# neka-nat/probreg

Hardware: NVIDIA H100
Metric: cpd_em_iterations_per_sec (higher is better)
Workload: dtype f32

## Files before the change

### probreg_b200/csrc/cpd_b200.cu

```cuda
#include "cpd_b200.h"
#include "kernels.cuh"
#include "lowrank.cuh"
#include "gram_i8.cuh"
#include "bcpd.cuh"
#include "gmmtree.cuh"
#include "l2dist.cuh"
#include "ocsvm.cuh"
#include "lattice.cuh"
#include "batch.cuh"

#include <cub/device/device_radix_sort.cuh>
#ifdef CPD_HOST_EMU
#include "emu_nccl.h"
#include "emu_solver.h"
#endif

#include <dlfcn.h>
#include <math.h>
#include <stdarg.h>
#include <stdio.h>
#include <stdlib.h>
#include <string.h>

#include <algorithm>
// ... 205 lines not shown
    DevBuf<float4> d_srcP, d_tgtP, d_tgtQ;
    DevBuf<P1Part> d_part1;
    DevBuf<double> d_part2;
    DevBuf<double> d_pt1, d_p1, d_pxc, d_px;
    DevBuf<double> d_mom_src, d_mom_tgt, d_mom, d_sums;
    DevBuf<DevState> d_state;
    DevState h_state;
    PinBuf<PinStage> pin;
    DevBuf<double> d_frame;
    PinBuf<double> h_stats;
    Event stats_ev, copy_ev;
    int stats_pending = 0;
    long long stats_count[2] = {0, 0};
    bool origin_given = false;
    int it1 = 0, it2 = 0, j1 = 1, j2 = 1, g1 = 1, g2 = 1;
    DevBuf<float4> d_sbox, d_tbox, d_ssub, d_tsub;
    DevBuf<float> d_omax, d_omax_sub;
    bool cull_on = true, cull_active = false;
    double extent = 0.0;
    DevBuf<int4> d_work1, d_work2;
    DevBuf<int> d_slots1, d_slots2;
    bool have_source = false, have_target = false, have_state = false, prepared = false;
    nccl_comm comm = nullptr;
    int world = 1, rank = 0;
    DevBuf<int> d_perm_src, d_perm_tgt, d_idx_tmp;
    DevBuf<unsigned> d_codes, d_codes_out;
    DevBuf<unsigned char> d_sort_tmp;
    DevBuf<double> d_outN, d_outM;
    DevBuf<float> d_G;
    DevBuf<double> d_W, d_A, d_B, d_ts2, d_nrpart;
    DevBuf<int64_t> d_ipiv;
    DevBuf<int> d_info;
    DevBuf<unsigned char> d_work;
// ... 63 lines not shown
    DevBuf<unsigned char> d_flush;
    std::vector<Event> pool;
};

namespace {
constexpr int STATE_RING = 8;
inline void drop_graph(cpd_ctx* h) {
#ifndef CPD_HOST_EMU
    h->em_graph.reset();
#endif
    (void)h;
}

inline unsigned blocks_for(long long n) { return (unsigned)((n + THREADS - 1) / THREADS); }

struct WorkList {
    std::vector<int4> items;
    std::vector<int> tile_slots;
    int max_slots = 1;
};
WorkList build_work(int ntiles, int nunits, int slots, double last_cost, double overhead) {
    const double OVERHEAD = overhead;
    WorkList w;
    nunits = std::max(1, nunits);
    auto cost_of = [&](int t) { return t == ntiles - 1 ? last_cost : 1.0; };
    auto span_of = [&](int t, int j) { return cost_of(t) * (double)((nunits + j - 1) / j) + OVERHEAD; };
    int best_j = 1;
    double best = 1e300;
    for (int j = 1; j <= nunits; ++j) {
        const long long items = (long long)ntiles * j;
// ... 121 lines not shown
        const double* t = h->h_stats.p + 9;
        if (!h->origin_given) for (int a = 0; a < 3; ++a) h->h_state.cx[a] = t[a] / (double)h->stats_count[1];
        h->extent = std::max(t[6] - t[3], std::max(t[7] - t[4], t[8] - t[5]));
    }
    h->stats_pending = 0;
    return CPD_OK;
}

int prepare(cpd_ctx* h) {
    TRY(ensure_stats(h));
    if (h->prepared) return CPD_OK;
    if (!h->have_source || !h->have_target) return fail(CPD_ERR_STATE, "source and target must both be set");
    h->it1 = (int)((h->n + ITILE1 - 1) / ITILE1);
    h->it2 = (int)((h->m + ITILE2 - 1) / ITILE2);
    const long long in_last = h->n - (long long)(h->it1 - 1) * ITILE1;
    const int live = (int)((in_last + 32 * RI1 - 1) / (32 * RI1));
    double last_cost = live < THREADS / 32 ? std::max(0.6, live / (double)(THREADS / 32)) : 1.0;
    if (const char* e = getenv("CPD_B200_PLAN_LAST_COST")) { const double v = atof(e); if (v > 0.0 && v <= 1.0) last_cost = v; }
    WorkList w1;
    if (const char* e = getenv("CPD_B200_PLAN_UNIT"); e && !strcmp(e, "stage")) {
        w1 = build_work(h->it1, (int)(h->mpad / P1_STAGE), h->slots1, last_cost, 0.5);
        for (int4& it : w1.items) { it.y *= P1_STAGE / SUB; it.z *= P1_STAGE / SUB; }
    } else {
        w1 = build_work(h->it1, (int)(h->mpad / SUB), h->slots1, last_cost, 0.5 * (P1_STAGE / SUB));
    }
    const WorkList w2 = build_work(h->it2, (int)(h->npad / P2_STAGE), h->slots2, 1.0, 0.5);
    h->j1 = w1.max_slots; h->g1 = (int)w1.items.size();
    h->j2 = w2.max_slots; h->g2 = (int)w2.items.size();
    TRY(h->d_work1.alloc(w1.items.size()));
    TRY(h->d_work2.alloc(w2.items.size()));
    TRY(h->d_slots1.alloc(w1.tile_slots.size()));
    TRY(h->d_slots2.alloc(w2.tile_slots.size()));
    CU(cudaMemcpyAsync(h->d_work1.p, w1.items.data(), w1.items.size() * sizeof(int4), cudaMemcpyHostToDevice, h->stream));
    CU(cudaMemcpyAsync(h->d_work2.p, w2.items.data(), w2.items.size() * sizeof(int4), cudaMemcpyHostToDevice, h->stream));
    CU(cudaMemcpyAsync(h->d_slots1.p, w1.tile_slots.data(), w1.tile_slots.size() * sizeof(int), cudaMemcpyHostToDevice, h->stream));
    CU(cudaMemcpyAsync(h->d_slots2.p, w2.tile_slots.data(), w2.tile_slots.size() * sizeof(int), cudaMemcpyHostToDevice, h->stream));
    CU(cudaStreamSynchronize(h->stream));
    TRY(h->d_sbox.alloc((size_t)(h->mpad / P1_STAGE) * 2));
    TRY(h->d_tbox.alloc((size_t)(h->npad / P2_STAGE) * 2));
    TRY(h->d_omax.alloc((size_t)(h->npad / P2_STAGE)));
    TRY(h->d_ssub.alloc((size_t)(h->mpad / SUB) * 2));
    TRY(h->d_tsub.alloc((size_t)(h->npad / SUB) * 2));
    TRY(h->d_omax_sub.alloc((size_t)(h->npad / SUB)));
    const size_t need1 = (size_t)h->j1 * h->n, need2 = (size_t)h->j2 * h->m * 4;
    TRY(h->d_part1.reserve(need1));
    TRY(h->d_part2.reserve(need2));
    const size_t ms = (size_t)blocks_for(h->m) * MOM_SRC, mt = (size_t)blocks_for(h->npad) * MOM_TGT;
    TRY(h->d_mom_src.reserve(ms));
    TRY(h->d_mom_tgt.reserve(mt));
    h->prepared = true;
    drop_graph(h);
    return CPD_OK;
}

int allreduce(cpd_ctx* h, double* buf, size_t count) {
// ... 7 lines not shown
}

int launch_estep(cpd_ctx* h, const double* d_sigma2, const double* d_w, const double* d_ts) {
    TRY(prepare(h));
    const long long cover = std::max(h->mpad, h->n);
    mark(h, 0);
    pack_kernel<<<blocks_for(cover), THREADS, 0, h->stream>>>(h->d_state.p, d_sigma2, h->d_yc.p, d_ts, h->d_xc.p, h->m, h->mpad,
                                                              h->n, h->d_srcP.p, h->d_tgtP.p);
    mark(h, 1);
    const bool cull = h->cull_on && h->cull_active;
    const int nst1 = (int)(h->mpad / P1_STAGE);
    stage_bbox_kernel<<<(unsigned)nst1, THREADS, 0, h->stream>>>(h->d_srcP.p, (int)h->m, P1_STAGE, h->d_sbox.p);
    h->launches += 1;
    const int nsub1 = (int)(h->mpad / SUB), nsub2 = (int)(h->npad / SUB);
    if (cull) {
        stage_bbox_kernel<<<(unsigned)(h->npad / P2_STAGE), THREADS, 0, h->stream>>>(h->d_tgtP.p, (int)h->n, P2_STAGE, h->d_tbox.p);
        sub_bbox_kernel<<<(unsigned)((nsub1 + 7) / 8), THREADS, 0, h->stream>>>(h->d_srcP.p, (int)h->m, nsub1, h->d_ssub.p);
        sub_bbox_kernel<<<(unsigned)((nsub2 + 7) / 8), THREADS, 0, h->stream>>>(h->d_tgtP.p, (int)h->n, nsub2, h->d_tsub.p);
        h->launches += 3;
    }
    const bool wgt = h->wgt_on;
    if (wgt) {
        weight_patch_kernel<<<blocks_for(h->m), THREADS, 0, h->stream>>>(h->d_la.p, h->m, h->d_srcP.p);
        h->launches += 1;
    }
#define CPD_PASS1(C, W) pass1_kernel<C, W><<<h->g1, THREADS, PASS1_SMEM, h->stream>>>(h->d_tgtP.p, (int)h->n, h->d_srcP.p, h->d_work1.p, h->d_part1.p, h->d_sbox.p, nst1, (C) ? h->d_ssub.p : nullptr)
    if (cull) { if (wgt) CPD_PASS1(true, true); else CPD_PASS1(true, false); }
    else { if (wgt) CPD_PASS1(false, true); else CPD_PASS1(false, false); }
#undef CPD_PASS1
    mark(h, 2);
    finalize1_kernel<<<blocks_for(h->npad), THREADS, 0, h->stream>>>(h->d_state.p, d_sigma2, d_w, h->d_part1.p, h->d_slots1.p, (int)h->n,
                                                                     h->d_tgtP.p, h->d_tgtQ.p, h->npad, h->d_pt1.p, h->d_mom_tgt.p,
                                                                     wgt ? h->d_log2c.p : nullptr);
    mark(h, 3);
    if (cull) {
        stage_omax_kernel<<<(unsigned)(h->npad / P2_STAGE), THREADS, 0, h->stream>>>(h->d_tgtQ.p, h->d_omax.p);
        sub_omax_kernel<<<(unsigned)((nsub2 + 7) / 8), THREADS, 0, h->stream>>>(h->d_tgtQ.p, nsub2, h->d_omax_sub.p);
        h->launches += 2;
    }
#define CPD_PASS2(C, W) pass2_kernel<C, W><<<h->g2, THREADS, PASS2_SMEM, h->stream>>>(h->d_srcP.p, (int)h->m, h->d_tgtQ.p, h->d_work2.p, h->d_part2.p, (C) ? h->d_tbox.p : nullptr, (C) ? h->d_omax.p : nullptr, (C) ? h->d_tsub.p : nullptr, (C) ? h->d_omax_sub.p : nullptr)
    if (cull) { if (wgt) CPD_PASS2(true, true); else CPD_PASS2(true, false); }
    else { if (wgt) CPD_PASS2(false, true); else CPD_PASS2(false, false); }
#undef CPD_PASS2
    mark(h, 4);
    finalize2_kernel<<<blocks_for(h->m), THREADS, 0, h->stream>>>(h->d_state.p, d_sigma2, h->d_part2.p, h->d_slots2.p, (int)h->m, h->d_yc.p,
                                                                  d_ts, h->d_p1.p, h->d_pxc.p, h->d_mom_src.p);
    mark(h, 5);
    mark(h, 6);
    KCHECK();
    h->launches += 5;
    return CPD_OK;
}

int read_params(cpd_ctx* h, cpd_params* out) {
    const DevState& s = h->pin.p->state;
    CU(cudaMemcpyAsync(&h->pin.p->state, h->d_state.p, sizeof(DevState), cudaMemcpyDeviceToHost, h->stream));
    CU(cudaStreamSynchronize(h->stream));
    if (s.err)
        return fail(CPD_ERR_STATE, "a peer rank did not deliver its moments within the P2P exchange timeout");
    const int d = h->dim;
    for (int i = 0; i < 9; ++i) out->lin[i] = 0.0;
    for (int i = 0; i < d; ++i)
        for (int j = 0; j < d; ++j) out->lin[i * d + j] = s.lin[3 * i + j];
    for (int i = 0; i < 3; ++i) out->t[i] = (i < d) ? s.t[i] : 0.0;
    out->scale = s.scale;
    out->sigma2 = s.sigma2;
    TRY(ensure_stats(h));
    h->cull_active = h->extent > 0.0 && 13.3 * sqrt(out->sigma2) < 0.25 * h->extent;
    out->q = s.q;
    out->n_p = s.n_p;
    return CPD_OK;
}
}

extern "C" int cpd_plan_work(int ntiles, int nunits, int slots, double last_tile_cost, int* items ,
                             int capacity, int* n_items, int* max_slots) {
    if (ntiles < 1 || nunits < 1 || slots < 1 || !(last_tile_cost > 0.0 && last_tile_cost <= 1.0) || !n_items || !max_slots)
        return fail(CPD_ERR_ARG, "bad argument");
    const WorkList w = build_work(ntiles, nunits, slots, last_tile_cost, 0.5 * (P1_STAGE / SUB));
    *n_items = (int)w.items.size();
    *max_slots = w.max_slots;
    if (items) {
        if (capacity < (int)w.items.size()) return fail(CPD_ERR_ARG, "capacity %d < %d work items", capacity, (int)w.items.size());
// ... 20 lines not shown
        return fail(CPD_ERR_CUDA, "device %d is sm_%d%d; this library is built for sm_90a (Hopper) only", device, prop.major, prop.minor);
    std::unique_ptr<cpd_ctx> h(new cpd_ctx());
    h->device = device;
    h->dim = dim;
    h->sm_count = prop.multiProcessorCount;
    if (stream) h->stream = (cudaStream_t)stream;
    else { CU(cudaStreamCreateWithFlags(&h->owned_stream.s, cudaStreamNonBlocking)); h->stream = h->owned_stream.s; }
    CU(cudaFuncSetAttribute(pass1_kernel<false, false>, cudaFuncAttributeMaxDynamicSharedMemorySize, PASS1_SMEM));
    CU(cudaFuncSetAttribute(pass2_kernel<false, false>, cudaFuncAttributeMaxDynamicSharedMemorySize, PASS2_SMEM));
    CU(cudaFuncSetAttribute(pass1_kernel<true, false>, cudaFuncAttributeMaxDynamicSharedMemorySize, PASS1_SMEM));
    CU(cudaFuncSetAttribute(pass2_kernel<true, false>, cudaFuncAttributeMaxDynamicSharedMemorySize, PASS2_SMEM));
    CU(cudaFuncSetAttribute(pass1_kernel<false, true>, cudaFuncAttributeMaxDynamicSharedMemorySize, PASS1_SMEM));
    CU(cudaFuncSetAttribute(pass2_kernel<false, true>, cudaFuncAttributeMaxDynamicSharedMemorySize, PASS2_SMEM));
    CU(cudaFuncSetAttribute(pass1_kernel<true, true>, cudaFuncAttributeMaxDynamicSharedMemorySize, PASS1_SMEM));
    CU(cudaFuncSetAttribute(pass2_kernel<true, true>, cudaFuncAttributeMaxDynamicSharedMemorySize, PASS2_SMEM));
    int occ1 = 0, occ2 = 0;
    CU(cudaOccupancyMaxActiveBlocksPerMultiprocessor(&occ1, pass1_kernel<false, false>, THREADS, PASS1_SMEM));
    CU(cudaOccupancyMaxActiveBlocksPerMultiprocessor(&occ2, pass2_kernel<false, false>, THREADS, PASS2_SMEM));
    h->slots1 = h->sm_count * std::max(1, occ1);
    h->slots2 = h->sm_count * std::max(1, occ2);
    TRY(h->d_state.alloc(1));
    TRY(h->d_mom.alloc((size_t)MOM_PAD));
    TRY(h->pin.alloc(1));
    TRY(h->d_frame.alloc(16));
    TRY(h->h_stats.alloc(18));
    CU(cudaEventCreateWithFlags(&h->stats_ev.e, cudaEventDisableTiming));
    CU(cudaEventCreateWithFlags(&h->copy_ev.e, cudaEventDisableTiming));
    CU(cudaEventCreate(&h->ev0.e));
    CU(cudaEventCreate(&h->ev1.e));
    for (Event& e : h->sev) CU(cudaEventCreate(&e.e));
    { const char* e = getenv("CPD_B200_NO_CULL"); h->cull_on = !(e && e[0] == '1'); }
    { const char* e = getenv("CPD_B200_NO_GRAPH"); h->graph_on = !(e && e[0] == '1'); }
    memset(&h->h_state, 0, sizeof(DevState));
    h->h_state.dim = dim;
    h->h_state.scale = 1.0;
    h->h_state.lin[0] = h->h_state.lin[4] = h->h_state.lin[8] = 1.0;
    h->h_state.update_scale = 1;
    TRY(upload_state(h.get()));
    *out = h.release();
    return CPD_OK;
}

extern "C" void cpd_destroy(cpd_ctx* h) {
    if (!h) return;
    cudaSetDevice(h->device);
    cudaStreamSynchronize(h->stream);
// ... 83 lines not shown
    CU(cudaSetDevice(h->device));
    DevState& s = h->h_state;
    const int d = h->dim;
    for (int i = 0; i < 3; ++i)
        for (int j = 0; j < 3; ++j) s.lin[3 * i + j] = (i < d && j < d) ? init->lin[i * d + j] : (i == j ? 1.0 : 0.0);
    for (int i = 0; i < 3; ++i) s.t[i] = (i < d) ? init->t[i] : 0.0;
    s.scale = (tf_kind == CPD_TF_RIGID) ? init->scale : 1.0;
    s.sigma2 = init->sigma2;
    s.q = init->q;
    s.n_p = 0.0;
    s.w = w;
    s.tf_kind = tf_kind;
    s.update_scale = update_scale ? 1 : 0;
    s.dim = d;
    TRY(ensure_stats(h));
    h->cull_active = h->extent > 0.0 && 13.3 * sqrt(init->sigma2) < 0.25 * h->extent;
    h->have_state = true;
    return upload_state(h);
}

namespace {
int em_step_launches(cpd_ctx* h) {
    TRY(launch_estep(h, &h->d_state.p->sigma2, &h->d_state.p->w, nullptr));
    const int nbs = (int)blocks_for(h->m), nbt = (int)blocks_for(h->npad);
    if (h->d_p2p.p) {
        moments_p2p_kernel<<<1, 256, 0, h->stream>>>(h->d_state.p, h->d_mom_src.p, nbs, RM_SRC, h->d_mom_tgt.p, nbt, RM_TGT, h->d_mom.p,
                                                     h->d_p2p.p);
        h->launches += 1;
    } else if (h->comm) {
        moments_kernel<0><<<1, 256, 0, h->stream>>>(h->d_state.p, h->d_mom_src.p, nbs, RM_SRC, h->d_mom_tgt.p, nbt, RM_TGT, h->d_mom.p);
        TRY(allreduce(h, h->d_mom.p, MOM_PAD));
// ... 69 lines not shown
    if (iters_run) *iters_run = it;
    return CPD_OK;
}

extern "C" int cpd_estep(cpd_ctx* h, const double* t_source, double sigma2, double w, double* pt1, double* p1, double* px, double* n_p) {
    if (!h || !t_source) return fail(CPD_ERR_ARG, "null argument");
    if (!(sigma2 > 0.0)) return fail(CPD_ERR_ARG, "sigma2 must be positive, got %g", sigma2);
    if (!(w >= 0.0 && w < 1.0)) return fail(CPD_ERR_ARG, "w must be in [0, 1), got %g", w);
    if (!h->have_source || !h->have_target) return fail(CPD_ERR_STATE, "source and target must both be set");
    CU(cudaSetDevice(h->device));
    TRY(h->d_raw.reserve((size_t)h->m * 3));
    TRY(upload_cloud(h, t_source, h->m, h->d_raw.p));
    gather3_kernel<<<blocks_for(h->m), THREADS, 0, h->stream>>>(h->d_raw.p, h->d_perm_src.p, h->m, 0.0, 0.0, 0.0, h->d_ts.p);
    h->launches += 1;
    TRY(ensure_stats(h));
    h->cull_active = h->extent > 0.0 && 13.3 * sqrt(sigma2) < 0.25 * h->extent;
    h->pin.p->es[0] = sigma2;
    h->pin.p->es[1] = w;
    CU(cudaMemcpyAsync(&h->d_state.p->es_sigma2, h->pin.p->es, 2 * sizeof(double), cudaMemcpyHostToDevice, h->stream));
    TRY(launch_estep(h, &h->d_state.p->es_sigma2, &h->d_state.p->es_w, h->d_ts.p));
    if (h->comm) {
        TRY(allreduce(h, h->d_p1.p, (size_t)h->m));
        TRY(allreduce(h, h->d_pxc.p, (size_t)h->m * 3));
    }
    return cpd_last_estep(h, pt1, p1, px, n_p);
}

namespace {
int bcpd_weights(cpd_ctx* h, const double* alpha, const double* sdiag, const int* perm, const double* ssw) {
    const long long m = h->m;
    const unsigned nb = blocks_for(m);
// ... 30 lines not shown
    }
    if (!any_weight) return fail(CPD_ERR_ARG, "every source has zero weight");
    TRY(ensure_weight_buffers(h));
    h->pin.p->bc_ssw[0] = scale;
    h->pin.p->bc_ssw[1] = sigma2;
    h->pin.p->bc_ssw[2] = w;
    CU(cudaMemcpyAsync(h->d_bc_es.p, h->pin.p->bc_ssw, 3 * sizeof(double), cudaMemcpyHostToDevice, h->stream));
    CU(cudaMemcpyAsync(h->d_outM.p, alpha, (size_t)m * sizeof(double), cudaMemcpyHostToDevice, h->stream));
    CU(cudaMemcpyAsync(h->d_outM.p + m, sigma_diag, (size_t)m * sizeof(double), cudaMemcpyHostToDevice, h->stream));
    TRY(bcpd_weights(h, h->d_outM.p, h->d_outM.p + m, h->d_perm_src.p, h->d_bc_es.p));
    TRY(h->d_raw.reserve((size_t)m * 3));
    TRY(upload_cloud(h, t_source, m, h->d_raw.p));
    gather3_kernel<<<blocks_for(m), THREADS, 0, h->stream>>>(h->d_raw.p, h->d_perm_src.p, m, 0.0, 0.0, 0.0, h->d_ts.p);
    h->launches += 1;
    TRY(ensure_stats(h));
    h->cull_active = h->extent > 0.0 && 13.3 * sqrt(sigma2) < 0.25 * h->extent;
    h->pin.p->es[0] = sigma2;
    h->pin.p->es[1] = w;
    CU(cudaMemcpyAsync(&h->d_state.p->es_sigma2, h->pin.p->es, 2 * sizeof(double), cudaMemcpyHostToDevice, h->stream));
    h->wgt_on = true;
    const int r = launch_estep(h, &h->d_state.p->es_sigma2, &h->d_state.p->es_w, h->d_ts.p);
    h->wgt_on = false;
    TRY(r);
    if (h->comm) {
        TRY(allreduce(h, h->d_p1.p, (size_t)m));
        TRY(allreduce(h, h->d_pxc.p, (size_t)m * 3));
    }
    return cpd_last_estep(h, nu_d, nu, px, n_p);
}

extern "C" int cpd_last_estep(cpd_ctx* h, double* pt1, double* p1, double* px, double* n_p) {
// ... 78 lines not shown
```

### probreg_b200/csrc/kernels.cuh

```cuda
#pragma once
#include <cuda_runtime.h>
#include <stdint.h>

namespace cpd {

#ifndef CPD_RI1
#define CPD_RI1 4
#endif
#ifndef CPD_RI2
#define CPD_RI2 4
#endif
#ifndef CPD_MINB1
#define CPD_MINB1 2
#endif
#ifndef CPD_MINB2
#define CPD_MINB2 2
#endif
#ifndef CPD_UNROLL1
#define CPD_UNROLL1 4
#endif
#ifndef CPD_UNROLL2
#define CPD_UNROLL2 4
#endif
#ifndef CPD_SUB
#define CPD_SUB 64
#endif
#ifndef CPD_GRP
#define CPD_GRP 8
#endif
constexpr int UNROLL1 = CPD_UNROLL1, UNROLL2 = CPD_UNROLL2;
constexpr int THREADS = 256;
constexpr int RI1 = CPD_RI1, RI2 = CPD_RI2;
constexpr int ITILE1 = THREADS * RI1, ITILE2 = THREADS * RI2;
#ifndef CPD_P1_STAGE
#define CPD_P1_STAGE 512
#endif
#ifndef CPD_P2_STAGE
#define CPD_P2_STAGE 512
#endif
constexpr int P1_STAGE = CPD_P1_STAGE;
constexpr int P2_STAGE = CPD_P2_STAGE;
static_assert(P1_STAGE % 256 == 0 && P2_STAGE % 256 == 0 && P1_STAGE >= 256 && P2_STAGE >= 256, "stage sizes are multiples of 256");
constexpr int P1_REC = 16, P2_REC = 32;
#ifndef CPD_NSTAGE
#define CPD_NSTAGE 3
#endif
constexpr int NSTAGE = CPD_NSTAGE;
constexpr int P1_STAGE_BYTES = P1_STAGE * P1_REC, P2_STAGE_BYTES = P2_STAGE * P2_REC;
// ... 195 lines not shown
        }
        srcP[i] = o;
    }
    if (i < n) {
        tgtP[i] = make_float4((float)(sk * xc[3 * i]), (float)(sk * xc[3 * i + 1]), (float)(sk * xc[3 * i + 2]), 0.0f);
    }
}

__global__ void __launch_bounds__(THREADS)
weight_patch_kernel(const float* __restrict__ la, long long m, float4* __restrict__ srcP) {
    const long long i = (long long)blockIdx.x * THREADS + threadIdx.x;
    if (i < m) srcP[i].w = la[i];
}

constexpr float CULL_GAP = 130.0f;
__global__ void __launch_bounds__(THREADS)
stage_bbox_kernel(const float4* __restrict__ pts, int n, int blk, float4* __restrict__ box) {
    __shared__ float sh[6][THREADS / 32];
    const int b = blockIdx.x;
    float lo[3] = {3.0e38f, 3.0e38f, 3.0e38f}, hi[3] = {-3.0e38f, -3.0e38f, -3.0e38f};
    for (int i = b * blk + threadIdx.x; i < min(n, (b + 1) * blk); i += THREADS) {
        const float4 p = pts[i];
        lo[0] = fminf(lo[0], p.x); lo[1] = fminf(lo[1], p.y); lo[2] = fminf(lo[2], p.z);
        hi[0] = fmaxf(hi[0], p.x); hi[1] = fmaxf(hi[1], p.y); hi[2] = fmaxf(hi[2], p.z);
    }
    const int lane = threadIdx.x & 31, wid = threadIdx.x >> 5;
#pragma unroll
    for (int a = 0; a < 3; ++a) {
#pragma unroll
        for (int o = 16; o > 0; o >>= 1) {
// ... 2 lines not shown
        }
        if (lane == 0) { sh[a][wid] = lo[a]; sh[3 + a][wid] = hi[a]; }
    }
    __syncthreads();
    if (threadIdx.x == 0) {
        float l[3], h[3];
        for (int a = 0; a < 3; ++a) {
            l[a] = sh[a][0]; h[a] = sh[3 + a][0];
            for (int w = 1; w < THREADS / 32; ++w) { l[a] = fminf(l[a], sh[a][w]); h[a] = fmaxf(h[a], sh[3 + a][w]); }
        }
        box[2 * b] = make_float4(l[0], l[1], l[2], 0.f);
        box[2 * b + 1] = make_float4(h[0], h[1], h[2], 0.f);
    }
}
__global__ void __launch_bounds__(THREADS)
stage_omax_kernel(const float4* __restrict__ tgtQ, float* __restrict__ omax) {
    __shared__ float sh[THREADS / 32];
    const int b = blockIdx.x;
    float m = 3.0e38f;
    for (int i = threadIdx.x; i < P2_STAGE; i += THREADS) m = fminf(m, tgtQ[2 * ((size_t)b * P2_STAGE + i)].w);
#pragma unroll
    for (int o = 16; o > 0; o >>= 1) m = fminf(m, __shfl_xor_sync(0xffffffffu, m, o));
    if ((threadIdx.x & 31) == 0) sh[threadIdx.x >> 5] = m;
    __syncthreads();
    if (threadIdx.x == 0) {
        for (int w = 1; w < THREADS / 32; ++w) m = fminf(m, sh[w]);
        omax[b] = -m;
    }
}
__global__ void __launch_bounds__(THREADS)
sub_bbox_kernel(const float4* __restrict__ pts, int n, int nsub, float4* __restrict__ box) {
    const int b = blockIdx.x * (THREADS / 32) + (threadIdx.x >> 5), lane = threadIdx.x & 31;
    if (b >= nsub) return;
    float lo[3] = {3.0e38f, 3.0e38f, 3.0e38f}, hi[3] = {-3.0e38f, -3.0e38f, -3.0e38f};
    for (int i = b * SUB + lane; i < min(n, (b + 1) * SUB); i += 32) {
        const float4 p = pts[i];
        lo[0] = fminf(lo[0], p.x); lo[1] = fminf(lo[1], p.y); lo[2] = fminf(lo[2], p.z);
        hi[0] = fmaxf(hi[0], p.x); hi[1] = fmaxf(hi[1], p.y); hi[2] = fmaxf(hi[2], p.z);
    }
#pragma unroll
    for (int a = 0; a < 3; ++a) {
#pragma unroll
        for (int o = 16; o > 0; o >>= 1) {
            lo[a] = fminf(lo[a], __shfl_xor_sync(0xffffffffu, lo[a], o));
            hi[a] = fmaxf(hi[a], __shfl_xor_sync(0xffffffffu, hi[a], o));
// ... 3 lines not shown
        box[2 * b] = make_float4(lo[0], lo[1], lo[2], 0.f);
        box[2 * b + 1] = make_float4(hi[0], hi[1], hi[2], 0.f);
    }
}
__global__ void __launch_bounds__(THREADS)
sub_omax_kernel(const float4* __restrict__ tgtQ, int nsub, float* __restrict__ omax) {
    const int b = blockIdx.x * (THREADS / 32) + (threadIdx.x >> 5), lane = threadIdx.x & 31;
    if (b >= nsub) return;
    float m = 3.0e38f;
    for (int i = lane; i < SUB; i += 32) m = fminf(m, tgtQ[2 * ((size_t)b * SUB + i)].w);
#pragma unroll
    for (int o = 16; o > 0; o >>= 1) m = fminf(m, __shfl_xor_sync(0xffffffffu, m, o));
    if (lane == 0) omax[b] = -m;
}
template <int RI>
__device__ __forceinline__ void warp_bbox(const float (&ax)[RI], const float (&ay)[RI], const float (&az)[RI], float* __restrict__ wbox) {
    float lo[3] = {3.0e38f, 3.0e38f, 3.0e38f}, hi[3] = {-3.0e38f, -3.0e38f, -3.0e38f};
#pragma unroll
    for (int r = 0; r < RI; ++r) {
        lo[0] = fminf(lo[0], ax[r]); hi[0] = fmaxf(hi[0], ax[r]);
        lo[1] = fminf(lo[1], ay[r]); hi[1] = fmaxf(hi[1], ay[r]);
        lo[2] = fminf(lo[2], az[r]); hi[2] = fmaxf(hi[2], az[r]);
    }
#pragma unroll
    for (int a = 0; a < 3; ++a) {
#pragma unroll
        for (int o = 16; o > 0; o >>= 1) {
            lo[a] = fminf(lo[a], __shfl_xor_sync(0xffffffffu, lo[a], o));
            hi[a] = fmaxf(hi[a], __shfl_xor_sync(0xffffffffu, hi[a], o));
        }
    }
// ... 9 lines not shown
    const float gz = fmaxf(0.f, fmaxf(blo.z - wbox[5], wbox[2] - bhi.z));
    return fmaf(gz, gz, fmaf(gy, gy, gx * gx)) * 0.9999f;
}

template <bool WGT>
__device__ __forceinline__ float pass1_t(const float ax, const float ay, const float az, const float no, const float4 b) {
    const float dx = __fsub_rn(ax, b.x), dy = __fsub_rn(ay, b.y), dz = __fsub_rn(az, b.z);
    float t = __fmaf_rn(dz, dz, __fmaf_rn(dy, dy, __fmaf_rn(dx, dx, no)));
    if (WGT) t = __fadd_rn(t, b.w);
    return t;
}
template <bool WGT>
__device__ __forceinline__ void pass1_sum(const float4* __restrict__ q, const float (&ax)[RI1], const float (&ay)[RI1],
                                          const float (&az)[RI1], const float (&no)[RI1], float (&Sc)[RI1], float (&Uc)[RI1]) {
    if (GRP > 0) {
#pragma unroll 1
        for (int g0 = 0; g0 < SUB; g0 += (GRP > 0 ? GRP : SUB)) {
            float gs[RI1], gu[RI1];
#pragma unroll
            for (int r = 0; r < RI1; ++r) {
#pragma unroll
                for (int jj = 0; jj < (GRP > 0 ? GRP : 1); ++jj) {
                    const float t = pass1_t<WGT>(ax[r], ay[r], az[r], no[r], q[g0 + jj]);
                    const float e = ex2(-t);
                    gs[r] = jj == 0 ? e : __fadd_rn(gs[r], e);
                    gu[r] = jj == 0 ? __fmul_rn(e, t) : __fmaf_rn(e, t, gu[r]);
                }
            }
#pragma unroll
            for (int r = 0; r < RI1; ++r) { Sc[r] = __fadd_rn(Sc[r], gs[r]); Uc[r] = __fadd_rn(Uc[r], gu[r]); }
        }
// ... 8 lines not shown
                Sc[r] = __fadd_rn(Sc[r], e);
                Uc[r] = __fmaf_rn(e, t, Uc[r]);
            }
        }
    }
}
template <bool WGT>
__device__ __forceinline__ float pass1_u(const float ax, const float ay, const float az, const float4 b) {
    const float dx = __fsub_rn(ax, b.x), dy = __fsub_rn(ay, b.y), dz = __fsub_rn(az, b.z);
    float u = __fmaf_rn(dz, dz, __fmaf_rn(dy, dy, __fmul_rn(dx, dx)));
    if (WGT) u = __fadd_rn(u, b.w);
    return u;
}

template <bool CULL, bool WGT>
__global__ void __launch_bounds__(THREADS, CPD_MINB1)
pass1_kernel(const float4* __restrict__ ipts, int ni, const float4* __restrict__ jrec, const int4* __restrict__ work,
             P1Part* __restrict__ part, const float4* __restrict__ sbox ,
             int nstages_total, const float4* __restrict__ ssub ) {
    __shared__ float wbox[THREADS / 32][8];
    CPD_DYN_SMEM(smraw);
    uint64_t* full = reinterpret_cast<uint64_t*>(smraw + NSTAGE * P1_STAGE_BYTES);
    const int tid = threadIdx.x;
    const int4 wk = work[blockIdx.x];
    constexpr int SPS = P1_STAGE / SUB;
    const int itile = wk.x, split = wk.w;
    const int st0 = wk.y / SPS, nst = (wk.z + SPS - 1) / SPS - st0;
    const int sc_first = wk.y - st0 * SPS, sc_last = wk.z - (st0 + nst - 1) * SPS;
    const unsigned char* jbytes = reinterpret_cast<const unsigned char*>(jrec);
    if (tid == 0) {
        for (int s = 0; s < NSTAGE; ++s) mbar_init(&full[s], 1);
        mbar_fence_init();
    }
    __syncthreads();
    if (tid == 0) {
// ... 1 lines not shown
            mbar_expect_tx(&full[s], P1_STAGE_BYTES);
            tma_load_1d(smraw + s * P1_STAGE_BYTES, jbytes + (size_t)(st0 + s) * P1_STAGE_BYTES, P1_STAGE_BYTES, &full[s]);
        }
    }
    if (itile * ITILE1 + (tid >> 5) * (32 * RI1) >= ni) return;
    float ax[RI1], ay[RI1], az[RI1], no[RI1];
    double S[RI1], SU[RI1];
#pragma unroll
    for (int r = 0; r < RI1; ++r) {
        int n = itile * ITILE1 + (tid >> 5) * (32 * RI1) + r * 32 + (tid & 31);
        n = n < ni ? n : ni - 1;
        const float4 p = ipts[n];
        ax[r] = p.x; ay[r] = p.y; az[r] = p.z;
        no[r] = -O_INIT;
    }
    float* const mybox = wbox[tid >> 5];
    warp_bbox<RI1>(ax, ay, az, mybox);
    {
        const int lane = tid & 31;
        float best = 3.0e38f;
        int bi = 0;
        for (int sidx = lane; sidx < nstages_total; sidx += 32) {
            const float g2 = box_gap2(mybox, sbox[2 * sidx], sbox[2 * sidx + 1]);
            if (g2 < best) { best = g2; bi = sidx; }
        }
#pragma unroll
        for (int o = 16; o > 0; o >>= 1) {
            const float ob = __shfl_xor_sync(0xffffffffu, best, o);
            const int oi = __shfl_xor_sync(0xffffffffu, bi, o);
            if (ob < best || (ob == best && oi < bi)) { best = ob; bi = oi; }
        }
        const float4* near = jrec + (size_t)bi * P1_STAGE;
        float cm[RI1];
#pragma unroll
        for (int r = 0; r < RI1; ++r) cm[r] = 3.0e38f;
#pragma unroll 4
        for (int jj = 0; jj < 128; ++jj) {
            const float4 b = near[jj];
#pragma unroll
            for (int r = 0; r < RI1; ++r) cm[r] = fminf(cm[r], pass1_u<WGT>(ax[r], ay[r], az[r], b));
        }
#pragma unroll
        for (int r = 0; r < RI1; ++r) no[r] = -fminf(O_INIT, floorf(cm[r]));
    }
    float omax_w = O_INIT;
    if (CULL) {
        float om = -3.0e38f;
#pragma unroll
        for (int r = 0; r < RI1; ++r) om = fmaxf(om, -no[r]);
#pragma unroll
        for (int o = 16; o > 0; o >>= 1) om = fmaxf(om, __shfl_xor_sync(0xffffffffu, om, o));
        omax_w = om;
    }
#pragma unroll
    for (int r = 0; r < RI1; ++r) { S[r] = 0.0; SU[r] = 0.0; }
    for (int it = 0; it < nst; ++it) {
        const int s = it % NSTAGE;
        mbar_wait(&full[s], (uint32_t)((it / NSTAGE) & 1));
        const float4* sp = reinterpret_cast<const float4*>(smraw + s * P1_STAGE_BYTES);
        bool skip = false;
        if (CULL) {
            const float4 blo = sbox[2 * (st0 + it)], bhi = sbox[2 * (st0 + it) + 1];
            skip = box_gap2(mybox, blo, bhi) - omax_w >= CULL_GAP;
        }
#pragma unroll 1
        for (int sc = (it == 0 ? sc_first : 0); sc < (skip ? 0 : (it == nst - 1 ? sc_last : SPS)); ++sc) {
            if (CULL) {
                const int sb = (st0 + it) * (P1_STAGE / SUB) + sc;
                if (box_gap2(mybox, ssub[2 * sb], ssub[2 * sb + 1]) - omax_w >= CULL_GAP) continue;
            }
            const float4* q = sp + sc * SUB;
            float Sc[RI1], Uc[RI1];
#pragma unroll
            for (int r = 0; r < RI1; ++r) { Sc[r] = 0.0f; Uc[r] = 0.0f; }
            pass1_sum<WGT>(q, ax, ay, az, no, Sc, Uc);
            bool bad = false;
#pragma unroll
            for (int r = 0; r < RI1; ++r) bad |= !(Sc[r] < TWO100);
            if (__any_sync(0xffffffffu, bad)) {
                float cm[RI1];
#pragma unroll
                for (int r = 0; r < RI1; ++r) cm[r] = 3.0e38f;
#pragma unroll UNROLL1
                for (int jj = 0; jj < SUB; ++jj) {
                    const float4 b = q[jj];
#pragma unroll
                    for (int r = 0; r < RI1; ++r) cm[r] = fminf(cm[r], pass1_u<WGT>(ax[r], ay[r], az[r], b));
                }
#pragma unroll
                for (int r = 0; r < RI1; ++r) {
                    const float o = -no[r], on = fminf(o, floorf(cm[r]));
                    const int sh = (int)fmaxf(on - o, -4000.0f);
                    S[r] = ldexp(S[r], sh); SU[r] = ldexp(SU[r], sh);
                    no[r] = -on;
                    Sc[r] = 0.0f; Uc[r] = 0.0f;
                }
                if (CULL) {
                    float om = -3.0e38f;
#pragma unroll
                    for (int r = 0; r < RI1; ++r) om = fmaxf(om, -no[r]);
#pragma unroll
                    for (int o = 16; o > 0; o >>= 1) om = fmaxf(om, __shfl_xor_sync(0xffffffffu, om, o));
                    omax_w = om;
                }
                pass1_sum<WGT>(q, ax, ay, az, no, Sc, Uc);
            }
#pragma unroll
            for (int r = 0; r < RI1; ++r) {
                S[r] += (double)Sc[r];
                SU[r] += (double)Uc[r] - (double)no[r] * (double)Sc[r];
            }
        }
        __syncthreads();
        if (tid == 0 && it + NSTAGE < nst) {
            mbar_expect_tx(&full[s], P1_STAGE_BYTES);
            tma_load_1d(smraw + s * P1_STAGE_BYTES, jbytes + (size_t)(st0 + it + NSTAGE) * P1_STAGE_BYTES, P1_STAGE_BYTES, &full[s]);
        }
    }
// ... 75 lines not shown
        finalize_column(log2S, c, lc, dead_shift, omin, SU, p1n, no, rnf, srr);
        pt1[i] = p1n;
        const float4 b = tgtP[i];
        v[0] = srr;
        v[1] = p1n;
        tgtQ[2 * (size_t)i] = make_float4(b.x, b.y, b.z, no);
        tgtQ[2 * (size_t)i + 1] = make_float4(rnf, 0.f, 0.f, 0.f);
    } else if (i < npad) {
        tgtQ[2 * (size_t)i] = make_float4(0.f, 0.f, 0.f, INFINITY);
        tgtQ[2 * (size_t)i + 1] = make_float4(0.f, 0.f, 0.f, 0.f);
    }
    block_reduce_store<RM_TGT>(v, mom_part + (size_t)blockIdx.x * RM_TGT);
}

template <bool CULL, bool WGT>
__global__ void __launch_bounds__(THREADS, CPD_MINB2)
pass2_kernel(const float4* __restrict__ ipts, int ni, const float4* __restrict__ jrec, const int4* __restrict__ work,
             double* __restrict__ part , const float4* __restrict__ tbox ,
             const float* __restrict__ omax_stage, const float4* __restrict__ tsub, const float* __restrict__ omax_sub) {
    __shared__ float wbox[THREADS / 32][8];
    CPD_DYN_SMEM(smraw);
    uint64_t* full = reinterpret_cast<uint64_t*>(smraw + NSTAGE * P2_STAGE_BYTES);
    const int tid = threadIdx.x;
    const int4 wk = work[blockIdx.x];
    const int itile = wk.x, st0 = wk.y, split = wk.w;
    const int nst = wk.z - wk.y;
    const unsigned char* jbytes = reinterpret_cast<const unsigned char*>(jrec);
    if (tid == 0) {
        for (int s = 0; s < NSTAGE; ++s) mbar_init(&full[s], 1);
        mbar_fence_init();
    }
    __syncthreads();
    if (tid == 0) {
        for (int s = 0; s < NSTAGE && s < nst; ++s) {
            mbar_expect_tx(&full[s], P2_STAGE_BYTES);
// ... 5 lines not shown
#pragma unroll
    for (int r = 0; r < RI2; ++r) {
        int m = itile * ITILE2 + (tid >> 5) * (32 * RI2) + r * 32 + (tid & 31);
        m = m < ni ? m : ni - 1;
        const float4 p = ipts[m];
        ax[r] = p.x; ay[r] = p.y; az[r] = p.z; al[r] = p.w;
    }
    float* const mybox = wbox[tid >> 5];
    if (CULL) warp_bbox<RI2>(ax, ay, az, mybox);
#pragma unroll
    for (int r = 0; r < RI2; ++r) { A1[r] = 0.0; AX[r] = 0.0; AY[r] = 0.0; AZ[r] = 0.0; }
    for (int it = 0; it < nst; ++it) {
        const int s = it % NSTAGE;
        mbar_wait(&full[s], (uint32_t)((it / NSTAGE) & 1));
        const float4* sp = reinterpret_cast<const float4*>(smraw + s * P2_STAGE_BYTES);
        bool skip = false;
        if (CULL) {
            const float4 blo = tbox[2 * (st0 + it)], bhi = tbox[2 * (st0 + it) + 1];
            skip = box_gap2(mybox, blo, bhi) - omax_stage[st0 + it] >= CULL_GAP;
        }
#pragma unroll 1
        for (int sc = 0; sc < (skip ? 0 : P2_STAGE / SUB); ++sc) {
            if (CULL) {
                const int sb = (st0 + it) * (P2_STAGE / SUB) + sc;
                if (box_gap2(mybox, tsub[2 * sb], tsub[2 * sb + 1]) - omax_sub[sb] >= CULL_GAP) continue;
            }
            const float4* q = sp + sc * (2 * SUB);
            float s1[RI2], sx[RI2], sy[RI2], sz[RI2];
#pragma unroll
            for (int r = 0; r < RI2; ++r) { s1[r] = 0.0f; sx[r] = 0.0f; sy[r] = 0.0f; sz[r] = 0.0f; }
            if (GRP > 0) {
#pragma unroll (CULL && WGT) ? 1 : 2
                for (int g0 = 0; g0 < SUB; g0 += (GRP > 0 ? GRP : SUB)) {
                    float g1[RI2], gx[RI2], gy[RI2], gz[RI2];
#pragma unroll
                    for (int jj = 0; jj < (GRP > 0 ? GRP : 1); ++jj) {
                        const float4 b = q[2 * (g0 + jj)];
                        const float rn = q[2 * (g0 + jj) + 1].x;
#pragma unroll
                        for (int r = 0; r < RI2; ++r) {
                            const float dx = __fsub_rn(ax[r], b.x), dy = __fsub_rn(ay[r], b.y), dz = __fsub_rn(az[r], b.z);
                            float t = __fmaf_rn(dz, dz, __fmaf_rn(dy, dy, __fmaf_rn(dx, dx, b.w)));
                            if (WGT) t = __fadd_rn(t, al[r]);
                            const float pr = __fmul_rn(ex2(-t), rn);
                            g1[r] = jj == 0 ? pr : __fadd_rn(g1[r], pr);
                            gx[r] = jj == 0 ? __fmul_rn(pr, dx) : __fmaf_rn(pr, dx, gx[r]);
                            gy[r] = jj == 0 ? __fmul_rn(pr, dy) : __fmaf_rn(pr, dy, gy[r]);
// ... 935 lines not shown
```

Baseline: 113.3.

## Cull CPD E-step at per-group sub-chunk granularity with decoupled tile sizes

Splits each pass1 warp's points into 128-point offset groups, each with its own bounding box, omax, and selective rebasing. Sub-chunk culling for a stage is now tested in parallel, one lane per sub-chunk, and combined with a warp ballot. This replaces the stage-level bbox/omax kernels and the per-iteration serial tests in both passes. Tile size is decoupled from thread count, slot counts come from launch bounds instead of the occupancy query, and the culling threshold becomes a tunable ratio. These changes aim to skip more far-field work and remove launches, at the cost of more per-group bookkeeping and a changed threshold (0.027 versus the old 0.25/13.3 ≈ 0.0188) that turns culling on in more cases.

Result: no change. 113.4 (median of 6 runs) (+0.1%).

```diff
diff --git a/probreg_b200/csrc/cpd_b200.cu b/probreg_b200/csrc/cpd_b200.cu
--- a/probreg_b200/csrc/cpd_b200.cu
+++ b/probreg_b200/csrc/cpd_b200.cu
@@ -243,9 +243,10 @@
     long long stats_count[2] = {0, 0};
     bool origin_given = false;
     int it1 = 0, it2 = 0, j1 = 1, j2 = 1, g1 = 1, g2 = 1;
-    DevBuf<float4> d_sbox, d_tbox, d_ssub, d_tsub;
-    DevBuf<float> d_omax, d_omax_sub;
+    DevBuf<float4> d_sbox, d_ssub, d_tsub;
+    DevBuf<float> d_omax_sub;
     bool cull_on = true, cull_active = false;
+    double cull_ratio = CULL_SIGMA_PER_EXTENT;
     double extent = 0.0;
     DevBuf<int4> d_work1, d_work2;
     DevBuf<int> d_slots1, d_slots2;
@@ -339,6 +340,10 @@
 
 inline unsigned blocks_for(long long n) { return (unsigned)((n + THREADS - 1) / THREADS); }
 
+inline void set_culling(cpd_ctx* h, double sigma2) {
+    h->cull_active = h->extent > 0.0 && sqrt(sigma2) < h->cull_ratio * h->extent;
+}
+
 struct WorkList {
     std::vector<int4> items;
     std::vector<int> tile_slots;
@@ -490,8 +495,8 @@
     h->it1 = (int)((h->n + ITILE1 - 1) / ITILE1);
     h->it2 = (int)((h->m + ITILE2 - 1) / ITILE2);
     const long long in_last = h->n - (long long)(h->it1 - 1) * ITILE1;
-    const int live = (int)((in_last + 32 * RI1 - 1) / (32 * RI1));
-    double last_cost = live < THREADS / 32 ? std::max(0.6, live / (double)(THREADS / 32)) : 1.0;
+    const int live = (int)((in_last + GROUP1 - 1) / GROUP1);
+    double last_cost = live < ITILE1 / GROUP1 ? std::max(0.6, live / (double)(ITILE1 / GROUP1)) : 1.0;
     if (const char* e = getenv("CPD_B200_PLAN_LAST_COST")) { const double v = atof(e); if (v > 0.0 && v <= 1.0) last_cost = v; }
     WorkList w1;
     if (const char* e = getenv("CPD_B200_PLAN_UNIT"); e && !strcmp(e, "stage")) {
@@ -513,8 +518,6 @@
     CU(cudaMemcpyAsync(h->d_slots2.p, w2.tile_slots.data(), w2.tile_slots.size() * sizeof(int), cudaMemcpyHostToDevice, h->stream));
     CU(cudaStreamSynchronize(h->stream));
     TRY(h->d_sbox.alloc((size_t)(h->mpad / P1_STAGE) * 2));
-    TRY(h->d_tbox.alloc((size_t)(h->npad / P2_STAGE) * 2));
-    TRY(h->d_omax.alloc((size_t)(h->npad / P2_STAGE)));
     TRY(h->d_ssub.alloc((size_t)(h->mpad / SUB) * 2));
     TRY(h->d_tsub.alloc((size_t)(h->npad / SUB) * 2));
     TRY(h->d_omax_sub.alloc((size_t)(h->npad / SUB)));
@@ -552,17 +555,16 @@
     h->launches += 1;
     const int nsub1 = (int)(h->mpad / SUB), nsub2 = (int)(h->npad / SUB);
     if (cull) {
-        stage_bbox_kernel<<<(unsigned)(h->npad / P2_STAGE), THREADS, 0, h->stream>>>(h->d_tgtP.p, (int)h->n, P2_STAGE, h->d_tbox.p);
         sub_bbox_kernel<<<(unsigned)((nsub1 + 7) / 8), THREADS, 0, h->stream>>>(h->d_srcP.p, (int)h->m, nsub1, h->d_ssub.p);
         sub_bbox_kernel<<<(unsigned)((nsub2 + 7) / 8), THREADS, 0, h->stream>>>(h->d_tgtP.p, (int)h->n, nsub2, h->d_tsub.p);
-        h->launches += 3;
+        h->launches += 2;
     }
     const bool wgt = h->wgt_on;
     if (wgt) {
         weight_patch_kernel<<<blocks_for(h->m), THREADS, 0, h->stream>>>(h->d_la.p, h->m, h->d_srcP.p);
         h->launches += 1;
     }
-#define CPD_PASS1(C, W) pass1_kernel<C, W><<<h->g1, THREADS, PASS1_SMEM, h->stream>>>(h->d_tgtP.p, (int)h->n, h->d_srcP.p, h->d_work1.p, h->d_part1.p, h->d_sbox.p, nst1, (C) ? h->d_ssub.p : nullptr)
+#define CPD_PASS1(C, W) pass1_kernel<C, W><<<h->g1, P1_THREADS, PASS1_SMEM, h->stream>>>(h->d_tgtP.p, (int)h->n, h->d_srcP.p, h->d_work1.p, h->d_part1.p, h->d_sbox.p, nst1, (C) ? h->d_ssub.p : nullptr)
     if (cull) { if (wgt) CPD_PASS1(true, true); else CPD_PASS1(true, false); }
     else { if (wgt) CPD_PASS1(false, true); else CPD_PASS1(false, false); }
 #undef CPD_PASS1
@@ -572,11 +574,10 @@
                                                                      wgt ? h->d_log2c.p : nullptr);
     mark(h, 3);
     if (cull) {
-        stage_omax_kernel<<<(unsigned)(h->npad / P2_STAGE), THREADS, 0, h->stream>>>(h->d_tgtQ.p, h->d_omax.p);
         sub_omax_kernel<<<(unsigned)((nsub2 + 7) / 8), THREADS, 0, h->stream>>>(h->d_tgtQ.p, nsub2, h->d_omax_sub.p);
-        h->launches += 2;
-    }
-#define CPD_PASS2(C, W) pass2_kernel<C, W><<<h->g2, THREADS, PASS2_SMEM, h->stream>>>(h->d_srcP.p, (int)h->m, h->d_tgtQ.p, h->d_work2.p, h->d_part2.p, (C) ? h->d_tbox.p : nullptr, (C) ? h->d_omax.p : nullptr, (C) ? h->d_tsub.p : nullptr, (C) ? h->d_omax_sub.p : nullptr)
+        h->launches += 1;
+    }
+#define CPD_PASS2(C, W) pass2_kernel<C, W><<<h->g2, P2_THREADS, PASS2_SMEM, h->stream>>>(h->d_srcP.p, (int)h->m, h->d_tgtQ.p, h->d_work2.p, h->d_part2.p, (C) ? h->d_tsub.p : nullptr, (C) ? h->d_omax_sub.p : nullptr)
     if (cull) { if (wgt) CPD_PASS2(true, true); else CPD_PASS2(true, false); }
     else { if (wgt) CPD_PASS2(false, true); else CPD_PASS2(false, false); }
 #undef CPD_PASS2
@@ -604,7 +605,7 @@
     out->scale = s.scale;
     out->sigma2 = s.sigma2;
     TRY(ensure_stats(h));
-    h->cull_active = h->extent > 0.0 && 13.3 * sqrt(out->sigma2) < 0.25 * h->extent;
+    set_culling(h, out->sigma2);
     out->q = s.q;
     out->n_p = s.n_p;
     return CPD_OK;
@@ -655,11 +656,12 @@
     CU(cudaFuncSetAttribute(pass2_kernel<false, true>, cudaFuncAttributeMaxDynamicSharedMemorySize, PASS2_SMEM));
     CU(cudaFuncSetAttribute(pass1_kernel<true, true>, cudaFuncAttributeMaxDynamicSharedMemorySize, PASS1_SMEM));
     CU(cudaFuncSetAttribute(pass2_kernel<true, true>, cudaFuncAttributeMaxDynamicSharedMemorySize, PASS2_SMEM));
-    int occ1 = 0, occ2 = 0;
-    CU(cudaOccupancyMaxActiveBlocksPerMultiprocessor(&occ1, pass1_kernel<false, false>, THREADS, PASS1_SMEM));
-    CU(cudaOccupancyMaxActiveBlocksPerMultiprocessor(&occ2, pass2_kernel<false, false>, THREADS, PASS2_SMEM));
-    h->slots1 = h->sm_count * std::max(1, occ1);
-    h->slots2 = h->sm_count * std::max(1, occ2);
+    h->slots1 = h->sm_count * CPD_MINB1;
+    h->slots2 = h->sm_count * CPD_MINB2;
+    if (const char* e = getenv("CPD_B200_PLAN_SLOTS")) {
+        int a = 0, b = 0;
+        if (sscanf(e, "%d,%d", &a, &b) == 2 && a > 0 && b > 0) { h->slots1 = a; h->slots2 = b; }
+    }
     TRY(h->d_state.alloc(1));
     TRY(h->d_mom.alloc((size_t)MOM_PAD));
     TRY(h->pin.alloc(1));
@@ -671,6 +673,7 @@
     CU(cudaEventCreate(&h->ev1.e));
     for (Event& e : h->sev) CU(cudaEventCreate(&e.e));
     { const char* e = getenv("CPD_B200_NO_CULL"); h->cull_on = !(e && e[0] == '1'); }
+    if (const char* e = getenv("CPD_B200_CULL_RATIO")) { const double v = atof(e); if (v >= 0.0) h->cull_ratio = v; }
     { const char* e = getenv("CPD_B200_NO_GRAPH"); h->graph_on = !(e && e[0] == '1'); }
     memset(&h->h_state, 0, sizeof(DevState));
     h->h_state.dim = dim;
@@ -784,7 +787,7 @@
     s.update_scale = update_scale ? 1 : 0;
     s.dim = d;
     TRY(ensure_stats(h));
-    h->cull_active = h->extent > 0.0 && 13.3 * sqrt(init->sigma2) < 0.25 * h->extent;
+    set_culling(h, init->sigma2);
     h->have_state = true;
     return upload_state(h);
 }
@@ -884,7 +887,7 @@
     gather3_kernel<<<blocks_for(h->m), THREADS, 0, h->stream>>>(h->d_raw.p, h->d_perm_src.p, h->m, 0.0, 0.0, 0.0, h->d_ts.p);
     h->launches += 1;
     TRY(ensure_stats(h));
-    h->cull_active = h->extent > 0.0 && 13.3 * sqrt(sigma2) < 0.25 * h->extent;
+    set_culling(h, sigma2);
     h->pin.p->es[0] = sigma2;
     h->pin.p->es[1] = w;
     CU(cudaMemcpyAsync(&h->d_state.p->es_sigma2, h->pin.p->es, 2 * sizeof(double), cudaMemcpyHostToDevice, h->stream));
@@ -945,7 +948,7 @@
     gather3_kernel<<<blocks_for(m), THREADS, 0, h->stream>>>(h->d_raw.p, h->d_perm_src.p, m, 0.0, 0.0, 0.0, h->d_ts.p);
     h->launches += 1;
     TRY(ensure_stats(h));
-    h->cull_active = h->extent > 0.0 && 13.3 * sqrt(sigma2) < 0.25 * h->extent;
+    set_culling(h, sigma2);
     h->pin.p->es[0] = sigma2;
     h->pin.p->es[1] = w;
     CU(cudaMemcpyAsync(&h->d_state.p->es_sigma2, h->pin.p->es, 2 * sizeof(double), cudaMemcpyHostToDevice, h->stream));
diff --git a/probreg_b200/csrc/kernels.cuh b/probreg_b200/csrc/kernels.cuh
--- a/probreg_b200/csrc/kernels.cuh
+++ b/probreg_b200/csrc/kernels.cuh
@@ -28,10 +28,26 @@
 #ifndef CPD_GRP
 #define CPD_GRP 8
 #endif
+#ifndef CPD_GUNROLL1
+#define CPD_GUNROLL1 1
+#endif
+#ifndef CPD_GUNROLL2
+#define CPD_GUNROLL2 2
+#endif
 constexpr int UNROLL1 = CPD_UNROLL1, UNROLL2 = CPD_UNROLL2;
+constexpr int GUNROLL1 = CPD_GUNROLL1, GUNROLL2 = CPD_GUNROLL2;
 constexpr int THREADS = 256;
 constexpr int RI1 = CPD_RI1, RI2 = CPD_RI2;
-constexpr int ITILE1 = THREADS * RI1, ITILE2 = THREADS * RI2;
+#ifndef CPD_ITILE2
+#define CPD_ITILE2 1024
+#endif
+constexpr int ITILE1 = 1024, ITILE2 = CPD_ITILE2;
+constexpr int P1_THREADS = ITILE1 / RI1, P2_THREADS = ITILE2 / RI2;
+constexpr int GROUP1 = 128;
+constexpr int RG1 = GROUP1 / 32;
+constexpr int GPW1 = RI1 / RG1;
+static_assert(ITILE1 % RI1 == 0 && ITILE2 % RI2 == 0 && P1_THREADS % 32 == 0 && P2_THREADS % 32 == 0, "whole warps per tile");
+static_assert(RI1 % RG1 == 0, "a warp holds whole offset groups");
 #ifndef CPD_P1_STAGE
 #define CPD_P1_STAGE 512
 #endif
@@ -257,6 +273,7 @@
 }
 
 constexpr float CULL_GAP = 130.0f;
+constexpr double CULL_SIGMA_PER_EXTENT = 0.027;
 __global__ void __launch_bounds__(THREADS)
 stage_bbox_kernel(const float4* __restrict__ pts, int n, int blk, float4* __restrict__ box) {
     __shared__ float sh[6][THREADS / 32];
@@ -289,21 +306,6 @@
     }
 }
 __global__ void __launch_bounds__(THREADS)
-stage_omax_kernel(const float4* __restrict__ tgtQ, float* __restrict__ omax) {
-    __shared__ float sh[THREADS / 32];
-    const int b = blockIdx.x;
-    float m = 3.0e38f;
-    for (int i = threadIdx.x; i < P2_STAGE; i += THREADS) m = fminf(m, tgtQ[2 * ((size_t)b * P2_STAGE + i)].w);
-#pragma unroll
-    for (int o = 16; o > 0; o >>= 1) m = fminf(m, __shfl_xor_sync(0xffffffffu, m, o));
-    if ((threadIdx.x & 31) == 0) sh[threadIdx.x >> 5] = m;
-    __syncthreads();
-    if (threadIdx.x == 0) {
-        for (int w = 1; w < THREADS / 32; ++w) m = fminf(m, sh[w]);
-        omax[b] = -m;
-    }
-}
-__global__ void __launch_bounds__(THREADS)
 sub_bbox_kernel(const float4* __restrict__ pts, int n, int nsub, float4* __restrict__ box) {
     const int b = blockIdx.x * (THREADS / 32) + (threadIdx.x >> 5), lane = threadIdx.x & 31;
     if (b >= nsub) return;
@@ -337,7 +339,7 @@
     if (lane == 0) omax[b] = -m;
 }
 template <int RI>
-__device__ __forceinline__ void warp_bbox(const float (&ax)[RI], const float (&ay)[RI], const float (&az)[RI], float* __restrict__ wbox) {
+__device__ __forceinline__ void warp_bbox(const float* ax, const float* ay, const float* az, float* __restrict__ wbox) {
     float lo[3] = {3.0e38f, 3.0e38f, 3.0e38f}, hi[3] = {-3.0e38f, -3.0e38f, -3.0e38f};
 #pragma unroll
     for (int r = 0; r < RI; ++r) {
@@ -377,7 +379,7 @@
 __device__ __forceinline__ void pass1_sum(const float4* __restrict__ q, const float (&ax)[RI1], const float (&ay)[RI1],
                                           const float (&az)[RI1], const float (&no)[RI1], float (&Sc)[RI1], float (&Uc)[RI1]) {
     if (GRP > 0) {
-#pragma unroll 1
+#pragma unroll GUNROLL1
         for (int g0 = 0; g0 < SUB; g0 += (GRP > 0 ? GRP : SUB)) {
             float gs[RI1], gu[RI1];
 #pragma unroll
@@ -416,11 +418,12 @@
 }
 
 template <bool CULL, bool WGT>
-__global__ void __launch_bounds__(THREADS, CPD_MINB1)
+__global__ void __launch_bounds__(P1_THREADS, CPD_MINB1)
 pass1_kernel(const float4* __restrict__ ipts, int ni, const float4* __restrict__ jrec, const int4* __restrict__ work,
              P1Part* __restrict__ part, const float4* __restrict__ sbox ,
              int nstages_total, const float4* __restrict__ ssub ) {
-    __shared__ float wbox[THREADS / 32][8];
+    static_assert(P1_STAGE / SUB <= 32 && P2_STAGE / SUB <= 32, "one lane per sub-chunk of a stage in the culling test");
+    __shared__ float gbox[P1_THREADS / 32 * GPW1][8];
     CPD_DYN_SMEM(smraw);
     uint64_t* full = reinterpret_cast<uint64_t*>(smraw + NSTAGE * P1_STAGE_BYTES);
     const int tid = threadIdx.x;
@@ -452,14 +455,16 @@
         ax[r] = p.x; ay[r] = p.y; az[r] = p.z;
         no[r] = -O_INIT;
     }
-    float* const mybox = wbox[tid >> 5];
-    warp_bbox<RI1>(ax, ay, az, mybox);
-    {
+    float* const mybox = gbox[(tid >> 5) * GPW1];
+#pragma unroll
+    for (int g = 0; g < GPW1; ++g) {
+        float* const box = mybox + 8 * g;
+        warp_bbox<RG1>(ax + g * RG1, ay + g * RG1, az + g * RG1, box);
         const int lane = tid & 31;
         float best = 3.0e38f;
         int bi = 0;
         for (int sidx = lane; sidx < nstages_total; sidx += 32) {
-            const float g2 = box_gap2(mybox, sbox[2 * sidx], sbox[2 * sidx + 1]);
+            const float g2 = box_gap2(box, sbox[2 * sidx], sbox[2 * sidx + 1]);
             if (g2 < best) { best = g2; bi = sidx; }
         }
 #pragma unroll
@@ -469,26 +474,31 @@
             if (ob < best || (ob == best && oi < bi)) { best = ob; bi = oi; }
         }
         const float4* near = jrec + (size_t)bi * P1_STAGE;
-        float cm[RI1];
-#pragma unroll
-        for (int r = 0; r < RI1; ++r) cm[r] = 3.0e38f;
+        float cm[RG1];
+#pragma unroll
+        for (int r = 0; r < RG1; ++r) cm[r] = 3.0e38f;
 #pragma unroll 4
         for (int jj = 0; jj < 128; ++jj) {
             const float4 b = near[jj];
 #pragma unroll
-            for (int r = 0; r < RI1; ++r) cm[r] = fminf(cm[r], pass1_u<WGT>(ax[r], ay[r], az[r], b));
-        }
-#pragma unroll
-        for (int r = 0; r < RI1; ++r) no[r] = -fminf(O_INIT, floorf(cm[r]));
-    }
-    float omax_w = O_INIT;
-    if (CULL) {
+            for (int r = 0; r < RG1; ++r) cm[r] = fminf(cm[r], pass1_u<WGT>(ax[g * RG1 + r], ay[g * RG1 + r], az[g * RG1 + r], b));
+        }
+#pragma unroll
+        for (int r = 0; r < RG1; ++r) no[g * RG1 + r] = -fminf(O_INIT, floorf(cm[r]));
+    }
+    float omax_g[GPW1];
+    auto group_omax = [&](int g) {
         float om = -3.0e38f;
 #pragma unroll
-        for (int r = 0; r < RI1; ++r) om = fmaxf(om, -no[r]);
+        for (int r = 0; r < RG1; ++r) om = fmaxf(om, -no[g * RG1 + r]);
 #pragma unroll
         for (int o = 16; o > 0; o >>= 1) om = fmaxf(om, __shfl_xor_sync(0xffffffffu, om, o));
-        omax_w = om;
+        omax_g[g] = om;
+    };
+#pragma unroll
+    for (int g = 0; g < GPW1; ++g) {
+        omax_g[g] = O_INIT;
+        if (CULL) group_omax(g);
     }
 #pragma unroll
     for (int r = 0; r < RI1; ++r) { S[r] = 0.0; SU[r] = 0.0; }
@@ -496,26 +506,37 @@
         const int s = it % NSTAGE;
         mbar_wait(&full[s], (uint32_t)((it / NSTAGE) & 1));
         const float4* sp = reinterpret_cast<const float4*>(smraw + s * P1_STAGE_BYTES);
-        bool skip = false;
+        unsigned live = ~0u;
         if (CULL) {
-            const float4 blo = sbox[2 * (st0 + it)], bhi = sbox[2 * (st0 + it) + 1];
-            skip = box_gap2(mybox, blo, bhi) - omax_w >= CULL_GAP;
+            const int lane = tid & 31;
+            bool far = false;
+            if (lane < SPS) {
+                const int sb = (st0 + it) * SPS + lane;
+                const float4 blo = ssub[2 * sb], bhi = ssub[2 * sb + 1];
+                far = true;
+#pragma unroll
+                for (int g = 0; g < GPW1; ++g) far &= box_gap2(mybox + 8 * g, blo, bhi) - omax_g[g] >= CULL_GAP;
+            }
+            live = ~__ballot_sync(0xffffffffu, far);
         }
 #pragma unroll 1
-        for (int sc = (it == 0 ? sc_first : 0); sc < (skip ? 0 : (it == nst - 1 ? sc_last : SPS)); ++sc) {
-            if (CULL) {
-                const int sb = (st0 + it) * (P1_STAGE / SUB) + sc;
-                if (box_gap2(mybox, ssub[2 * sb], ssub[2 * sb + 1]) - omax_w >= CULL_GAP) continue;
-            }
+        for (int sc = (it == 0 ? sc_first : 0); sc < (it == nst - 1 ? sc_last : SPS); ++sc) {
+            if (CULL && !((live >> sc) & 1u)) continue;
             const float4* q = sp + sc * SUB;
             float Sc[RI1], Uc[RI1];
 #pragma unroll
             for (int r = 0; r < RI1; ++r) { Sc[r] = 0.0f; Uc[r] = 0.0f; }
             pass1_sum<WGT>(q, ax, ay, az, no, Sc, Uc);
-            bool bad = false;
-#pragma unroll
-            for (int r = 0; r < RI1; ++r) bad |= !(Sc[r] < TWO100);
-            if (__any_sync(0xffffffffu, bad)) {
+            bool rebase[GPW1], any = false;
+#pragma unroll
+            for (int g = 0; g < GPW1; ++g) {
+                bool bad = false;
+#pragma unroll
+                for (int r = 0; r < RG1; ++r) bad |= !(Sc[g * RG1 + r] < TWO100);
+                rebase[g] = __any_sync(0xffffffffu, bad);
+                any |= rebase[g];
+            }
+            if (any) {
                 float cm[RI1];
 #pragma unroll
                 for (int r = 0; r < RI1; ++r) cm[r] = 3.0e38f;
@@ -527,19 +548,18 @@
                 }
 #pragma unroll
                 for (int r = 0; r < RI1; ++r) {
-                    const float o = -no[r], on = fminf(o, floorf(cm[r]));
-                    const int sh = (int)fmaxf(on - o, -4000.0f);
-                    S[r] = ldexp(S[r], sh); SU[r] = ldexp(SU[r], sh);
-                    no[r] = -on;
+                    if (rebase[r / RG1]) {
+                        const float o = -no[r], on = fminf(o, floorf(cm[r]));
+                        const int sh = (int)fmaxf(on - o, -4000.0f);
+                        S[r] = ldexp(S[r], sh); SU[r] = ldexp(SU[r], sh);
+                        no[r] = -on;
+                    }
                     Sc[r] = 0.0f; Uc[r] = 0.0f;
                 }
                 if (CULL) {
-                    float om = -3.0e38f;
-#pragma unroll
-                    for (int r = 0; r < RI1; ++r) om = fmaxf(om, -no[r]);
-#pragma unroll
-                    for (int o = 16; o > 0; o >>= 1) om = fmaxf(om, __shfl_xor_sync(0xffffffffu, om, o));
-                    omax_w = om;
+#pragma unroll
+                    for (int g = 0; g < GPW1; ++g)
+                        if (rebase[g]) group_omax(g);
                 }
                 pass1_sum<WGT>(q, ax, ay, az, no, Sc, Uc);
             }
@@ -645,11 +665,11 @@
 }
 
 template <bool CULL, bool WGT>
-__global__ void __launch_bounds__(THREADS, CPD_MINB2)
+__global__ void __launch_bounds__(P2_THREADS, CPD_MINB2)
 pass2_kernel(const float4* __restrict__ ipts, int ni, const float4* __restrict__ jrec, const int4* __restrict__ work,
-             double* __restrict__ part , const float4* __restrict__ tbox ,
-             const float* __restrict__ omax_stage, const float4* __restrict__ tsub, const float* __restrict__ omax_sub) {
-    __shared__ float wbox[THREADS / 32][8];
+             double* __restrict__ part , const float4* __restrict__ tsub ,
+             const float* __restrict__ omax_sub) {
+    __shared__ float wbox[P2_THREADS / 32][8];
     CPD_DYN_SMEM(smraw);
     uint64_t* full = reinterpret_cast<uint64_t*>(smraw + NSTAGE * P2_STAGE_BYTES);
     const int tid = threadIdx.x;
@@ -685,23 +705,25 @@
         const int s = it % NSTAGE;
         mbar_wait(&full[s], (uint32_t)((it / NSTAGE) & 1));
         const float4* sp = reinterpret_cast<const float4*>(smraw + s * P2_STAGE_BYTES);
-        bool skip = false;
+        unsigned live = ~0u;
         if (CULL) {
-            const float4 blo = tbox[2 * (st0 + it)], bhi = tbox[2 * (st0 + it) + 1];
-            skip = box_gap2(mybox, blo, bhi) - omax_stage[st0 + it] >= CULL_GAP;
+            const int lane = tid & 31;
+            bool far = false;
+            if (lane < P2_STAGE / SUB) {
+                const int sb = (st0 + it) * (P2_STAGE / SUB) + lane;
+                far = box_gap2(mybox, tsub[2 * sb], tsub[2 * sb + 1]) - omax_sub[sb] >= CULL_GAP;
+            }
+            live = ~__ballot_sync(0xffffffffu, far);
         }
 #pragma unroll 1
-        for (int sc = 0; sc < (skip ? 0 : P2_STAGE / SUB); ++sc) {
-            if (CULL) {
-                const int sb = (st0 + it) * (P2_STAGE / SUB) + sc;
-                if (box_gap2(mybox, tsub[2 * sb], tsub[2 * sb + 1]) - omax_sub[sb] >= CULL_GAP) continue;
-            }
+        for (int sc = 0; sc < P2_STAGE / SUB; ++sc) {
+            if (CULL && !((live >> sc) & 1u)) continue;
             const float4* q = sp + sc * (2 * SUB);
             float s1[RI2], sx[RI2], sy[RI2], sz[RI2];
 #pragma unroll
             for (int r = 0; r < RI2; ++r) { s1[r] = 0.0f; sx[r] = 0.0f; sy[r] = 0.0f; sz[r] = 0.0f; }
             if (GRP > 0) {
-#pragma unroll (CULL && WGT) ? 1 : 2
+#pragma unroll (CULL && WGT) ? 1 : GUNROLL2
                 for (int g0 = 0; g0 < SUB; g0 += (GRP > 0 ? GRP : SUB)) {
                     float g1[RI2], gx[RI2], gy[RI2], gz[RI2];
 #pragma unroll
```
